# 20171130/Equivariant-NN-Zoo

Measured on AMD Instinct MI355X. Metric: molecules/s forward+backward, QM9 config_energy batch, higher is better.
Workload: dtype f32

## Files before the change

equivariant-nn-zoo_amd/csrc/e3k_layer.hip:

```cpp
#include <cstdlib>
#include <cstring>
#include <new>
#include <vector>

#include "e3k_common.h"

namespace e3k {

__global__ __launch_bounds__(256) void gather_rows_kernel(const float* __restrict__ src, const int64_t* __restrict__ rows, int n_rows,
                                                          int width, float* __restrict__ dst) {
  const int i = blockIdx.x * 256 + threadIdx.x;
  if (i >= n_rows * width) return;
  const int r = i / width, c = i - r * width;
  dst[i] = src[rows[r] * width + c];
}

__global__ __launch_bounds__(256) void scatter_rows_kernel(const float* __restrict__ src, const int64_t* __restrict__ rows,
                                                           const int32_t* __restrict__ bounds, int n_rows, int width,
                                                           float* __restrict__ dst) {
  const int i = blockIdx.x * 256 + threadIdx.x;
  if (i >= n_rows * width) return;
  const int r = i / width, c = i - r * width;
  if (bounds[2 * r + 1] > 0) atomicAdd(dst + rows[r] * width + c, src[i]);
}
// ... 139 lines not shown
    g.add(L, LAST_FWD, r.h, r.w_last, r.use_table ? r.T : r.w, r.R);
    E3K_TRY(g.run(0, st));
  }
  if (r.use_table && !in_kernel_table(d, r)) {
    Timed t(L, E3K_PROF_RTABLE_FWD, st, r.R, r.E);
    E3K_TRY(e3k_rtable_interp_fwd(r.T, r.bin_perm, r.bin, r.bin_coef, r.E, r.knots, d.W, r.w, st));
  }
  return pack_table(L, r, st);
}

}

extern "C" int e3k_layer_create(const e3k_layer_desc* desc, e3k_layer** out) {
  if (!desc || !out || !desc->tp) return E3K_ERR_INVALID;
  if (desc->n_hidden < 1 || desc->n_hidden > 4) return E3K_ERR_UNSUPPORTED;
  if (desc->w_live < 0 || desc->n_live < 0 || desc->n_live > 8 || (desc->w_live > 0) != (desc->n_live > 0)) return E3K_ERR_INVALID;
  if (desc->w_live > 0) {
    if (!e3k_tp_scalar_supported(desc->tp) || (desc->w_live % 4) || desc->w_live > desc->W) return E3K_ERR_UNSUPPORTED;
    int sum = 0;
    for (int i = 0; i < desc->n_live; ++i) {
      if (desc->live_col[i] < 0 || desc->live_len[i] <= 0 || desc->live_col[i] + desc->live_len[i] > desc->W) return E3K_ERR_INVALID;
      sum += desc->live_len[i];
    }
    if (sum != desc->w_live) return E3K_ERR_INVALID;
  }
  e3k_layer* L = new (std::nothrow) e3k_layer();
  if (!L) return E3K_ERR_LAUNCH;
  L->d = *desc;
  const e3k_gemm_set* src[N_SETS] = {&desc->lin1_fwd, &desc->lin1_dgrad, &desc->lin1_dgrad_acc, &desc->lin1_wgrad, &desc->post_fwd,
                                     &desc->post_dgrad, &desc->post_wgrad, &desc->sc_fwd, &desc->sc_dgrad, &desc->sc_wgrad,
                                     &desc->last_fwd, &desc->last_dgrad, &desc->last_wgrad};
  for (int i = 0; i < N_SETS; ++i) {
    const e3k_gemm_set& gs = *src[i];
// ... 219 lines not shown
    }
    if (with_lin1 && need_lin1) g.add(L, LIN1_WGRAD, a->x_cf, a->gb_lin1, a->g_x1, a->N);
    return g.run(1, st, rider);
  };
  if (side3 != main && (need_post || want_sc)) {
    E3K_TRY(edge(L, 0, main, side3));
    E3K_TRY(weight_grads(true, false, side3));
    if (want_sc) E3K_TRY(keyed_weight_grads());
  }
  const bool fused_xw_s = a->fuse_xw && !fused_xw && need_x1 && !in_kernel_table(d, r) && need_radial_side && a->E > 0 && a->g_w && a->x1 &&
                          r.w && side == main;
  const bool rtable_timed = L->prof_cap > 0 && ((L->prof_mask >> E3K_PROF_RTABLE_BWD) & 1u);
  float* const g_T_rows = narrow ? a->g_T_live : a->g_T;
  auto spread_table_gradient = [&](void* st) -> int {
    if (!narrow) return E3K_OK;
    int32_t src_col[8];
    for (int i = 0, pos = 0; i < d.n_live; ++i) {
      src_col[i] = pos;
      pos += d.live_len[i];
    }
    return e3k_expand_columns(a->g_T_live, r.R, d.w_live, d.W, src_col, d.live_col, d.live_len, d.n_live, a->g_T, st);
  };
  const bool ride = fused_xw && r.use_table && side == main && side3 == main && !rtable_timed && a->g_T && a->table_ws &&
                    (r.have_rows || !(need_last || need_hidden || a->need_radial));
  if (need_x1) {
    if (!a->g_x1) return E3K_ERR_INVALID;
    if (!d.tp_bwd_x_overwrites && e3k::zero_fill(a->g_x1, sizeof(float) * a->N * d.d_x1, (hipStream_t)main))
      return E3K_ERR_LAUNCH;
    Timed t(L, E3K_PROF_TP_BWD_X, main, a->N, a->E);
    if (narrow) {
      E3K_TRY(e3k_tp_bwd_xw_scalar_ptable(d.tp, a->x1, r.P, d.W, d.live_col, r.erec_src, a->g_mid, a->src_ptr, a->N, a->E, a->g_x1, a->g_w,
                                          main));
    } else if (fused_xw) {
      E3K_TRY(e3k_tp_bwd_xw_ptable(d.tp, a->x1, r.P, r.erec_src, a->g_mid, a->src_ptr, a->N, a->E, a->g_x1, a->g_w, main));
    } else if (fused_xw_s) {
      E3K_TRY(e3k_tp_bwd_xw(d.tp, a->x1, a->sh, r.w, a->g_mid, a->dst, a->src_ptr, a->src_perm, a->N, a->E, a->g_x1, a->g_w, main));
    } else if (in_kernel_table(d, r) && r.P) {
      E3K_TRY(e3k_tp_bwd_x_ptable(d.tp, r.P, r.erec_src, a->g_mid, a->src_ptr, a->N, a->E, a->g_x1, main));
    } else if (in_kernel_table(d, r)) {
      E3K_TRY(e3k_tp_bwd_x_table(d.tp, a->sh, r.T, r.bin, r.bin_coef, a->g_mid, a->dst, a->src_ptr, a->src_perm, a->N, a->E, a->g_x1, main));
    } else {
      E3K_TRY(e3k_tp_bwd_x(d.tp, a->sh, r.w, a->g_mid, a->dst, a->src_ptr, a->src_perm, a->N, a->E, a->g_x1, main));
    }
  }
  if (need_radial_side && a->E > 0) {
    if (!a->g_w) return E3K_ERR_INVALID;
// ... 248 lines not shown
```

equivariant-nn-zoo_amd/csrc/e3k_tp_scalar.hip:

```cpp
#include "e3k_tp_body.h"

namespace e3k {

constexpr int kScalarMaxGroups = 8;
struct ScalarCols {
  int32_t w_live;
  int32_t table_off[kScalarMaxGroups];
};
template <int L1> struct ScalarSlot { static constexpr int Q = L1 == 0 ? 0 : (L1 == 1 ? 1 : 4); };
static_assert(Slots<0>::L2[ScalarSlot<0>::Q] == 0 && Slots<0>::L3[ScalarSlot<0>::Q] == 0, "slot table changed");
static_assert(Slots<1>::L2[ScalarSlot<1>::Q] == 1 && Slots<1>::L3[ScalarSlot<1>::Q] == 0, "slot table changed");
static_assert(Slots<2>::L2[ScalarSlot<2>::Q] == 2 && Slots<2>::L3[ScalarSlot<2>::Q] == 0, "slot table changed");

template <int L1>
__device__ __forceinline__ void tp_bwd_xw_scalar_body(const TpArgs& a, const e3k_tp_group& g, const int w_live, const int table_off,
                                                      const int node, const int u) {
  constexpr int D1 = 2 * L1 + 1, Q = ScalarSlot<L1>::Q;
  const int mul = g.mul;
  const int u4 = u * 4;
  const int goff4 = uniform(g.out_off[Q] * 4), woff4 = uniform(g.w_off[Q] * 4), toff4 = uniform(table_off * 4);
  const float cf = g.coeff[Q];
  const int row_g = a.d_mid * 4, row_t = a.W * 4, row_w = w_live * 4;
  float gx[D1], xs[D1];
  const float* __restrict__ xr = a.x + (int64_t)node * a.d_in + g.x_off;
// ... 31 lines not shown
#pragma unroll
  for (int i = 0; i < D1; ++i) (gxr + i * mul)[u] = gx[i];
}

__global__ __launch_bounds__(256) void tp_bwd_xw_scalar_kernel(TpArgs a, ScalarCols cols, const e3k_tp_group* __restrict__ groups,
                                                               const int2* __restrict__ gc, int n_gc) {
  E3K_TP_PROLOGUE
  (void)part;
  const int toff = cols.table_off[uniform(gcv.x)];
  const int l1 = g.l1;
  if (l1 == 0) tp_bwd_xw_scalar_body<0>(a, g, cols.w_live, toff, node, u);
  else if (l1 == 1) tp_bwd_xw_scalar_body<1>(a, g, cols.w_live, toff, node, u);
  else tp_bwd_xw_scalar_body<2>(a, g, cols.w_live, toff, node, u);
}

constexpr int kExpandMaxRanges = 8;
struct ExpandRanges {
  int32_t n;
  int32_t src[kExpandMaxRanges], dst[kExpandMaxRanges], len[kExpandMaxRanges];
};
__global__ __launch_bounds__(256) void expand_columns_kernel(const float* __restrict__ src, int64_t rows, int w_src, int w_dst,
                                                             ExpandRanges rg, float* __restrict__ dst) {
  const int q_dst = w_dst / 4;
  const int64_t i = (int64_t)blockIdx.x * 256 + threadIdx.x;
  if (i >= rows * q_dst) return;
  const int64_t r = i / q_dst;
  const int c = (int)(i - r * q_dst) * 4;
  float4 v = make_float4(0.f, 0.f, 0.f, 0.f);
  for (int k = 0; k < rg.n; ++k)
    if (c >= rg.dst[k] && c < rg.dst[k] + rg.len[k]) v = *reinterpret_cast<const float4*>(src + r * w_src + rg.src[k] + (c - rg.dst[k]));
  *reinterpret_cast<float4*>(dst + r * w_dst + c) = v;
// ... 81 lines not shown
```

equivariant-nn-zoo_amd/e3_layers_amd/backend/conv_native.py:

```python
from __future__ import annotations

import ctypes as C
import dataclasses
from typing import List, Optional

import torch

from .tuning import knob as _knob
from torch.autograd.function import once_differentiable

from . import lib as L
from . import memo, ops, radial_table

ENABLED = TP_TABLE_PACKED = TP_BWD_FUSED = 1
PROF_KINDS = {"tp_fwd": 0, "tp_bwd_x": 1, "tp_bwd_w": 2, "rtable_fwd": 3, "rtable_bwd": 4, "radial_last_fwd": 5}
_LAYERS: List["NativeLayer"] = []


MAX_ROUNDS = 4
LIVE_GRAD = _knob("E3K_LIVE_GRAD")
NARROW_MAX_GROUPS = 8


def _hits(lo: int, hi: int, ranges) -> bool:
    return any(lo < b and a < hi for a, b in ranges)


def _covers(instr, width: int) -> bool:
    return sum(w for _, w in {(ins.in_off, ins.mul_in * ins.dim) for ins in instr}) == width


@dataclasses.dataclass
class LiveSets:
    cols: tuple
    conv: list
    post: list
# ... 134 lines not shown
            w += [(g.w_off[q], g.mul) for q in live_q]
            if live_q:
                x1.append((g.x_off, g.x_off + (2 * g.l1 + 1) * g.mul))
        lin1 = [ins for ins in plan.lin1_spec.instr if _hits(ins.out_off, ins.out_off + ins.mul_out * ins.dim, x1)]
        return LiveSets(tuple(cols), conv, post, sc, mid, slots, w, sorted(set(x1)), lin1)

    def narrow(self, cols) -> Optional["NativeLayer"]:
        cols = tuple(cols)
        if cols in self.narrows:
            return self.narrows[cols]
        from ..nn.core import tp_slots

        plan, nl = self.plan, None
        ls = self.live_sets(cols)
        groups = plan.tp_plan.groups
        fits = (0 < len(ls.slots) <= NARROW_MAX_GROUPS and len({gi for gi, _ in ls.slots}) == len(ls.slots) and not plan.addend
                and all(tp_slots(groups[gi].l1)[q] == (groups[gi].l1, 0) and groups[gi].l1 <= 2 and groups[gi].mul % 64 == 0
                        for gi, q in ls.slots))
        if fits:
            live_groups, pos = [], 0
            for gi, q in ls.slots:
                g, n = groups[gi], L.TpGroup()
                n.l1, n.x_off, n.mul, n.mask = g.l1, g.x_off, g.mul, 1 << q
                for t in range(4):
                    n.y_off[t] = g.y_off[t]
                n.w_off[q], n.out_off[q], n.out_stride[q], n.coeff[q] = pos, g.out_off[q], g.out_stride[q], g.coeff[q]
                pos += g.mul
                live_groups.append(n)
            tp = plan.tp_plan
            pruned = dict(tp_plan=ops.TpPlan(live_groups, tp.d_in, tp.d_sh, pos, tp.d_mid),
                          post_spec=dataclasses.replace(plan.post_spec, instr=ls.post, in_covered=_covers(ls.post, plan.post_spec.d_in)),
                          lin1_spec=dataclasses.replace(plan.lin1_spec, instr=ls.lin1, in_covered=_covers(ls.lin1, plan.lin1_spec.d_in)))
            if plan.sc_spec is not None:
                live_sc = [ins for _, ins in ls.sc]
                pruned.update(sc_spec=dataclasses.replace(plan.sc_spec, instr=live_sc, in_covered=_covers(live_sc, plan.sc_spec.d_in)),
                              sc_m_off=tuple(plan.sc_m_off[j] for j, _ in ls.sc))
            np_ = plan.replace(**pruned)
            try:
                nl = NativeLayer(np_, narrow_of=self)
            except NotImplementedError:
                nl = None
        if nl is not None:
            d = nl.desc
            if plan.sc_spec is not None:
                kw = ops._kw_array(plan.sc_spec, plan.sc_m_off)
                nl.keep.append(kw)
                d.kw, d.n_kw = kw, len(plan.sc_spec.instr)
            d.post_in_covered = 1
            d.w_live, d.n_live = pos, len(ls.slots)
            for i, (off, mul) in enumerate(ls.w):
                d.live_col[i], d.live_len[i] = off, mul
            nl.live = ls
        self.narrows[cols] = nl
        return nl

    def _all(self):
        return [self] + [n for n in self.narrows.values() if n is not None]

    def profile(self, capacity: int, kinds=None) -> None:
        mask = 0xFFFFFFFF if kinds is None else sum(1 << PROF_KINDS[k] for k in kinds)
        for lay in self._all():
            lay.prof = (capacity, mask)
            for h in lay.handles.values():
                L.check(L.load().e3k_layer_profile_mask(h, capacity, mask), "e3k_layer_profile_mask")

    def profile_read(self, kind: str):
        out = []
# ... 535 lines not shown
                                  p_tab)
            ctx.cfg = (plan, topo, groups, bool(in_cf), bool(out_cf), fork, len(w_hidden), table, carve, rcarve, need_relayout)
            ctx.stack = stack
            ctx.attrs_shape = tuple(node_attrs.shape) if (has_sc and not have_m) else None
        ctx.addend_inplace = addend_inplace
        if addend_inplace:
            return y, addend
        return y

    @staticmethod
    def backward(ctx, gy, *unused):
        from . import conv_block

        plan, topo, groups, in_cf, out_cf, fork, n_hidden, table, carve, rcarve, need_relayout = ctx.cfg
        live_cols = memo.recall(gy, "live_cols") if (LIVE_GRAD and gy is not None) else None
        saved = ctx.saved_tensors
        x_in, edge_radial, sh, buf, rbuf, w, w_lin1, w_post, w_sc, w_last, t_keep, m_pre = saved[:12]
        conv_ext = None
        if ctx.addend_inplace:
            conv_ext, m_pre = m_pre, None
            if gy is None:
                gy = torch.zeros(conv_ext.shape[0], plan.gate_spec.out_dim, device=conv_ext.device, dtype=torch.float32)
        w_hidden = saved[12:12 + n_hidden]
        p_tab = saved[12 + n_hidden]
        need = ctx.needs_input_grad
        need_x, need_attrs, need_radial, need_sh = need[0], need[1], need[2], need[3]
        stack, need_pre = ctx.stack, need[12]
        have_m, need_m = m_pre is not None, need[13]
        need_addend = bool(plan.addend and need[13])
        p0 = 14
        need_lin1, need_post, need_sc, need_last = need[p0], need[p0 + 1], need[p0 + 2], need[p0 + 3]
        need_hidden = need[p0 + 4:]
        if stack:
            need_radial = need_last = False
            need_hidden = ()
        if torch.is_grad_enabled() or need_sh:
            raise RuntimeError(
                "the fused convolution block serves first-order training only (no gradient w.r.t. the spherical harmonics, "
                "no create_graph=True): MessagePassing takes the composed path for those by itself; set E3K_CONV_BLOCK=0 "
                "if this was reached another way")
        has_sc = plan.sc_spec is not None
        dev = gy.device
        n, e, r = gy.shape[0], sh.shape[0], edge_radial.shape[0]
        narrow = None
        if live_cols is not None:
            cand = native_layer(plan).narrow(live_cols)
            if cand is not None:
                cand.handle(dev)
                if (stack and need_pre and table is not None and p_tab is not None and w is None and (need_x or need_lin1) and e > 0
                        and gy.dtype == torch.float32 and gy.is_contiguous()):
                    narrow = cand
        layer = (narrow or native_layer(plan)).handle(dev)
        main = ops.current_stream(dev)
        fork = fork and not torch.cuda.is_current_stream_capturing()
        side = ops.side_stream(dev, 0) if fork else main
        side2 = ops.side_stream(dev, 1) if fork else main
        side3 = ops.side_stream(dev, 2) if (fork and ops.WGRAD_SIDE) else main
        gy = L.f32c(gy)
        lin1, post, last, sc = plan.lin1_spec, plan.post_spec, plan.last_spec, plan.sc_spec
        off = carve.off
        a = L.LayerBwdArgs()
        a.N, a.E = n, e
        a.in_cf, a.out_cf, a.fork = int(in_cf), int(out_cf), int(fork)
        a.need_x, a.need_attrs, a.need_radial = int(need_x), int(bool(need_attrs and has_sc)), int(need_radial)
        a.fuse_xw = 1
# ... 121 lines not shown
            with conv_block._on(side2, main):
                g_attrs = torch.empty(ctx.attrs_shape, device=dev, dtype=torch.float32)
            a.g_attrs = g_attrs.data_ptr()
        if need_radial:
            with conv_block._on(side, main):
                g_radial = torch.empty_like(edge_radial)
            a.g_radial = g_radial.data_ptr()
        if HOST_TIMING is not None:
            import time

            t_c = time.perf_counter()
            L.check(L.load().e3k_layer_bwd(layer, C.byref(a)), "e3k_layer_bwd")
            HOST_TIMING[3] += time.perf_counter() - t_c
        else:
            L.check(L.load().e3k_layer_bwd(layer, C.byref(a)), "e3k_layer_bwd")
        if fork:
            for st in (side, side2, side3):
                if st is not main:
                    work.record_stream(st)
            buf.record_stream(side)
            if side3 is not main:
                buf.record_stream(side3)
                if x_in is not None:
                    x_in.record_stream(side3)
            _record_once(sh, side)
        if "post" in rets or "lin1" in rets:
            conv_block._wait(main, side3)
        if "sc" in rets:
            conv_block._wait(main, side2)
        if "last" in rets or any(f"h{i}" in rets for i in range(n_hidden)):
# ... 15 lines not shown
```

equivariant-nn-zoo_amd/e3_layers_amd/backend/lib.py:

```python
from __future__ import annotations

import ctypes as C
import os
from typing import Optional, Sequence

import torch

from .tuning import knob as _knob

_HERE = os.path.dirname(os.path.abspath(__file__))
CSRC_DIR = os.path.normpath(os.path.join(_HERE, "..", "..", "csrc"))
LIB_PATH = _knob("E3K_LIB") or os.path.join(CSRC_DIR, "libe3k.so")

TP_MAXQ = 8


class GemmProblem(C.Structure):
    _fields_ = [
        ("A", C.c_void_p), ("A2", C.c_void_p), ("B", C.c_void_p), ("C", C.c_void_p), ("bias", C.c_void_p),
        ("row_index", C.c_void_p), ("group_dev", C.c_void_p),
        ("M1", C.c_int32), ("M2", C.c_int32), ("N", C.c_int32), ("K", C.c_int32),
        ("V", C.c_int32), ("accumulate", C.c_int32),
        ("a_r1", C.c_int64), ("a_r2", C.c_int64), ("a_k", C.c_int64),
        ("a2_r1", C.c_int64),
        ("b_k", C.c_int64), ("b_n", C.c_int64),
        ("c_r1", C.c_int64), ("c_r2", C.c_int64), ("c_n", C.c_int64),
        ("alpha", C.c_float), ("act", C.c_int32), ("act_cst", C.c_float), ("chain", C.c_int32),
    ]

# ... 35 lines not shown
    _fields_ = [("p", C.POINTER(GemmProblem)), ("n", C.c_int32), ("n_rounds", C.c_int32), ("round_start", C.c_int32 * 5),
                ("_pad", C.c_int32)]


class LayerDesc(C.Structure):
    _fields_ = ([("tp", C.c_void_p)]
                + [(k, GemmSet) for k in ("lin1_fwd", "lin1_dgrad", "lin1_dgrad_acc", "lin1_wgrad", "post_fwd", "post_dgrad",
                                          "post_wgrad", "sc_fwd", "sc_dgrad", "sc_wgrad", "last_fwd", "last_dgrad", "last_wgrad")]
                + [("gate", C.POINTER(GateSeg)), ("n_gate", C.c_int32), ("n_in_blocks", C.c_int32), ("in_blocks", C.POINTER(Block)),
                   ("kw", C.POINTER(KwInstr)), ("n_kw", C.c_int32), ("V", C.c_int32), ("ld_m", C.c_int64),
                   ("k0", C.c_int32), ("h", C.c_int32), ("n_hidden", C.c_int32), ("act", C.c_int32), ("cst", C.c_float),
                   ("alphas", C.c_float * 4)]
                + [(k, C.c_int32) for k in ("d_in", "d_x1", "d_mid", "d_conv", "d_out", "W", "post_in_covered", "sc_in_covered",
                                            "lin1_in_covered", "sc_out_covered", "post_out_covered", "tp_bwd_x_overwrites",
                                            "w_live", "n_live")]
                + [("live_col", C.c_int32 * 8), ("live_len", C.c_int32 * 8)])


class LayerRadial(C.Structure):
    _fields_ = [("R", C.c_int64), ("E", C.c_int64), ("use_table", C.c_int32), ("keep", C.c_int32), ("knots", C.c_int32),
                ("have_rows", C.c_int32), ("in_kernel", C.c_int32), ("packed", C.c_int32), ("radial", C.c_void_p), ("bin", C.c_void_p), ("bin_ptr", C.c_void_p), ("bin_perm", C.c_void_p),
                ("bin_coef", C.c_void_p), ("bin_seg", C.c_void_p), ("w_last", C.c_void_p), ("w_hidden", C.c_void_p * 4), ("h", C.c_void_p),
                ("z", C.c_void_p * 4), ("T", C.c_void_p), ("w", C.c_void_p), ("erec_dst", C.c_void_p), ("erec_src", C.c_void_p), ("P", C.c_void_p)]


class RadialStackItem(C.Structure):
    _fields_ = [("rad", LayerRadial), ("g_rows", C.c_void_p), ("gb_last", C.c_void_p), ("gb_hidden", C.c_void_p * 4),
                ("g_h", C.c_void_p), ("g_radial", C.c_void_p), ("g_slope", C.c_void_p), ("hp", C.c_void_p), ("g_hp", C.c_void_p)]


class SlopeCtx(C.Structure):
# ... 121 lines not shown
    "e3k_tp_plan_destroy": (None, [_P]),
    "e3k_tp_fwd": (C.c_int, [_P, _P, _P, _P, _P, _P, _P, _I64, _I64, _P, _P]),
    "e3k_tp_bwd_w": (C.c_int, [_P, _P, _P, _P, _P, _P, _P, _P, _I64, _I64, _P, _P, _P]),
    "e3k_tp_bwd_w_ordered": (C.c_int, [_P, _P, _P, _P, _P, _P, _P, _P, _I64, _I64, _P, _P, _P, _P]),
    "e3k_tp_bwd_x_overwrites": (C.c_int, [_P]),
    "e3k_tp_last_route": (C.c_char_p, []),
    "e3k_gemm_last_routes": (C.c_char_p, []),
    "e3k_tp_table_supported": (C.c_int, [_P]),
    "e3k_tp_fwd_table": (C.c_int, [_P, _P, _P, _P, _P, _P, _P, _P, _P, _I64, _I64, _P, _P]),
    "e3k_tp_bwd_x_table": (C.c_int, [_P, _P, _P, _P, _P, _P, _P, _P, _P, _I64, _I64, _P, _P]),
    "e3k_tp_fwd_ptable": (C.c_int, [_P, _P, _P, _P, _P, _I64, _I64, _P, _P]),
    "e3k_tp_bwd_x_ptable": (C.c_int, [_P, _P, _P, _P, _P, _I64, _I64, _P, _P]),
    "e3k_tp_bwd_xw_ptable": (C.c_int, [_P, _P, _P, _P, _P, _P, _I64, _I64, _P, _P, _P]),
    "e3k_tp_scalar_supported": (C.c_int, [_P]),
    "e3k_tp_bwd_xw_scalar_ptable": (C.c_int, [_P, _P, _P, _I32, C.POINTER(_I32), _P, _P, _P, _I64, _I64, _P, _P, _P]),
    "e3k_expand_columns": (C.c_int, [_P, _I64, _I32, _I32, C.POINTER(_I32), C.POINTER(_I32), C.POINTER(_I32), _I32, _P, _P]),
    "e3k_tp_bwd_xw": (C.c_int, [_P, _P, _P, _P, _P, _P, _P, _P, _I64, _I64, _P, _P, _P]),
    "e3k_tp_bwd_xe": (C.c_int, [_P, _P, _P, _P, _P, _P, _P, _P, _P, _I64, _I64, _P, _P, _P, _P, _P, _P]),
    "e3k_tp_edge_partials_floats": (C.c_int64, [_P, _I64]),
    "e3k_tp_bwd_xw_dual": (C.c_int, [_P, _P, _P, _P, _P, _P, _P, _P, _P, _P, _P, _P, _I64, _I64, _P, _P, _P, _P]),
    "e3k_edge_records": (C.c_int, [_P, _P, _P, _P, _P, _I32, _I64, _P, _P]),
    "e3k_tp_table2_supported": (C.c_int, [_P]),
    "e3k_tp_second_order_streamed_supported": (C.c_int, [_P]),
    "e3k_tp_bwd_e_table": (C.c_int, [_P, _P, _P, _P, _P, _P, _P, _P, _P, _P, _P, _I64, _I64, _P, _P, _P, _P, _P]),
    "e3k_tp_fwd_jvp_table": (C.c_int, [_P, _P, _P, _P, _P, _P, _P, _P, _P, _P, _P, _P, _P, _I64, _I64, _P, _P]),
    "e3k_tp_bwd_x_dual_table": (C.c_int, [_P, _P, _P, _P, _P, _P, _P, _P, _P, _P, _P, _P, _I64, _I64, _P, _P]),
    "e3k_tp_bwd_w_dual": (C.c_int, [_P, _P, _P, _P, _P, _P, _P, _P, _P, _I64, _I64, _P, _P]),
    "e3k_tp_bwd_x": (C.c_int, [_P, _P, _P, _P, _P, _P, _P, _I64, _I64, _P, _P]),
    "e3k_csr_workspace_ints": (C.c_int64, [_I64, _I64]),
    "e3k_csr_build": (C.c_int, [_P, _I64, _I64, _P, _P, _P, _P, _P, _P, _P, _P, _P]),
# ... 118 lines not shown
```

equivariant-nn-zoo_amd/e3_layers_amd/backend/tuning.py:

```python
from __future__ import annotations

import os
from typing import Dict, Tuple

KNOBS: Dict[str, Tuple[object, str, str]] = {
    "E3K_CONV_BLOCK": (1, "path", "a layer as one autograd node (backend/conv_block.py); 0: one autograd.Function per kernel (the definition)"),
    "E3K_FORCE_BLOCK": (1, "path", "force training: a layer as three autograd nodes on the value + slope tables (backend/conv_force.py); 0: composed per-edge path"),
    "E3K_GEMM_CHAIN": (1, "path", "a Linear's terms that add onto one block (an irrep feeding two outputs: the second was an accumulating launch of its own) run as ONE K-chained GEMM problem; 0: one round of launches per term"),
    "E3K_FORCE_EDGE_ATOMICS": (0, "path", "force block: 1 = g_sh / g_r accumulated with float atomics across a plan's groups (rounds 4-5: forces not bit-reproducible); 0 = per-item partials combined in a fixed order"),
    "E3K_BLOCK_ADDEND": (1, "path", "layers with un-keyed node attributes run as fused blocks with the self-connection handed in as addend"),
    "E3K_BLOCK_LOOK_AHEAD": (1, "path", "a forked layer issues the next layer's radial branch behind its own tensor product"),
    "E3K_CF_CHAIN": (1, "path", "consecutive MessagePassing layers hand their features over channel-fastest"),
    "E3K_RADIAL_STACK": (1, "path", "the radial MLPs of all layers on one edge embedding evaluated as one batch"),
    "E3K_KW_STACK": (1, "path", "the per-key self-connection weights of all layers formed as one batch"),
    "E3K_TP_TABLE": (1, "path", "table layers interpolate their path weights inside the tensor-product kernels, from the table packed into 12-byte Taylor records (no w[E, W]); 0: interpolation pass"),
    "E3K_LIVE_GRAD": (1, "path", "a layer whose incoming gradient is marked zero outside some columns (the Linear in front of a scalar head marks it) runs the backward of the live paths only (conv_native.NativeLayer.narrow); 0: always the dense backward"),
    "E3K_FWD_FORK": (1, "path", "0: one stream; 1: radial / self-connection / weight-gradient branches on side streams above the edge thresholds (never inside a graph capture)"),
    "E3K_WGRAD_SIDE": (1, "path", "sunk weight gradients of forked layers run on a side stream"),
    "E3K_FORK_MIN_EDGES": (25000, "threshold", "per-edge radial layers fork from this many edges (in units of a 1920-weight layer)"),
    "E3K_FORK_MIN_EDGES_TABLE": (60000, "threshold", "table layers fork from this many edges"),
    "E3K_STACK_MAX_EDGES": (50000, "threshold", "forked layers use the radial stack up to this many edges (one-stream layers: always)"),
    "E3K_KW_STACK_MAX_EDGES": (10 ** 9, "threshold", "keyed-weight stack up to this many edges (measured: no upper limit pays)"),
    "E3K_WGRAD_SIDE_MIN_ROWS": (2048, "threshold", "composed path: weight gradients move to the side stream from this many rows"),
    "E3K_KEY_MAX": (256, "threshold", "keyed self-connection for at most this many distinct attribute rows"),
    "E3K_RADIAL_TABLE": (1, "accuracy", "radial MLP on a knot table + cubic interpolation per edge (bound by the guard below); 0: per edge"),
    "E3K_RADIAL_KNOTS": (512, "accuracy", "target knot count over [0, r_max] (the spacing is the power of two at or below r_max / knots)"),
    "E3K_RADIAL_KNOTS_SLOPE": (512, "accuracy", "... of the value + slope tables of force training"),
    "E3K_RADIAL_KNOTS_MAX": (2048, "accuracy", "a guard whose bound passes the tolerance doubles both knot counts up to this; beyond it that MLP's table is switched off (= E3K_RADIAL_KNOTS: never refine)"),
    "E3K_RADIAL_TABLE_KEYED": (0, "path", "one knot table per value of a small categorical edge key beside the radius (config_diffusion's bond type); measured slower than the per-edge MLP for the 32-channel net it serves: off"),
    "E3K_RADIAL_MIN_EDGES_PER_KNOT": (4.0, "threshold", "the table applies from this many edges per table row"),
    "E3K_RADIAL_TABLE_TOL": (1e-6, "accuracy", "a-posteriori interpolation-error bound above which an MLP's table is switched off"),
# ... 39 lines not shown
```

include/e3k.h:

```cpp
#ifndef E3K_H
#define E3K_H

#include <stdint.h>

#ifdef __cplusplus
extern "C" {
#endif

#define E3K_OK 0
#define E3K_ERR_INVALID (-1)
#define E3K_ERR_LAUNCH (-2)
#define E3K_ERR_UNSUPPORTED (-3)

#define E3K_TP_MAXQ 8

const char* e3k_strerror(int code);
int e3k_version(void);
void e3k_tp_limits(int* l1max, int* l2max, int* l3max);

typedef struct {
  const float* A;
  const float* A2;
  const float* B;
  float* C;
  const float* bias;
  const int32_t* row_index;
  const int32_t* group_dev;
  int32_t M1, M2, N, K;
  int32_t V;
// ... 105 lines not shown
int e3k_tp_table_supported(const e3k_tp_plan* plan);
int e3k_tp_fwd_table(const e3k_tp_plan* plan, const float* x, const float* sh, const float* T, const int32_t* bin,
                     const float* coef, const int32_t* src, const int32_t* dst_ptr, const int32_t* dst_perm, int64_t N, int64_t E,
                     float* out, void* stream);
int e3k_tp_bwd_x_table(const e3k_tp_plan* plan, const float* sh, const float* T, const int32_t* bin, const float* coef,
                       const float* g_out, const int32_t* dst, const int32_t* src_ptr, const int32_t* src_perm, int64_t N,
                       int64_t E, float* g_x, void* stream);
int e3k_tp_fwd_ptable(const e3k_tp_plan* plan, const float* x, const void* P, const int32_t* erec_dst, const int32_t* dst_ptr,
                      int64_t N, int64_t E, float* out, void* stream);
int e3k_tp_bwd_x_ptable(const e3k_tp_plan* plan, const void* P, const int32_t* erec_src, const float* g_out, const int32_t* src_ptr,
                        int64_t N, int64_t E, float* g_x, void* stream);
int e3k_tp_bwd_xw_ptable(const e3k_tp_plan* plan, const float* x, const void* P, const int32_t* erec_src, const float* g_out,
                         const int32_t* src_ptr, int64_t N, int64_t E, float* g_x, float* g_w, void* stream);
int e3k_tp_scalar_supported(const e3k_tp_plan* plan);
int e3k_tp_bwd_xw_scalar_ptable(const e3k_tp_plan* plan, const float* x, const void* P, int32_t table_w, const int32_t* table_off,
                                const int32_t* erec_src, const float* g_out, const int32_t* src_ptr, int64_t N, int64_t E, float* g_x,
                                float* g_w, void* stream);
int e3k_expand_columns(const float* src, int64_t rows, int32_t w_src, int32_t w_dst, const int32_t* src_col, const int32_t* dst_col,
                       const int32_t* len, int32_t n_ranges, float* dst, void* stream);
int e3k_tp_bwd_xw(const e3k_tp_plan* plan, const float* x, const float* sh, const float* w, const float* g_out, const int32_t* dst,
                  const int32_t* src_ptr, const int32_t* src_perm, int64_t N, int64_t E, float* g_x, float* g_w, void* stream);
int e3k_tp_table2_supported(const e3k_tp_plan* plan);
int e3k_tp_second_order_streamed_supported(const e3k_tp_plan* plan);
int e3k_tp_bwd_e_table(const e3k_tp_plan* plan, const float* x, const float* sh, const float* T, const float* D,
                       const int32_t* bin, const float* coef, const float* g_out, const int32_t* src, const int32_t* dst_ptr,
                       const int32_t* dst_perm, int64_t N, int64_t E, float* g_sh, float* g_r, float* g_w, float* e_partials,
                       void* stream);
int64_t e3k_tp_edge_partials_floats(const e3k_tp_plan* plan, int64_t E);
int e3k_tp_fwd_jvp_table(const e3k_tp_plan* plan, const float* x, const float* x2, const float* sh, const float* sh2,
                         const float* T, const float* D, const int32_t* bin, const float* coef, const float* s2,
// ... 281 lines not shown
  e3k_gemm_set sc_fwd, sc_dgrad, sc_wgrad;
  e3k_gemm_set last_fwd, last_dgrad, last_wgrad;
  const e3k_gate_seg* gate;
  int32_t n_gate;
  int32_t n_in_blocks;
  const e3k_block* in_blocks;
  const e3k_kw_instr* kw;
  int32_t n_kw, V;
  int64_t ld_m;
  int32_t k0, h, n_hidden, act;
  float cst;
  float alphas[4];
  int32_t d_in, d_x1, d_mid, d_conv, d_out, W;
  int32_t post_in_covered, sc_in_covered, lin1_in_covered, sc_out_covered, post_out_covered, tp_bwd_x_overwrites;
  int32_t w_live, n_live;
  int32_t live_col[8], live_len[8];
} e3k_layer_desc;

typedef struct e3k_layer e3k_layer;
int e3k_layer_create(const e3k_layer_desc* desc, e3k_layer** out);
void e3k_layer_destroy(e3k_layer* layer);

typedef struct {
  int64_t R, E;
  int32_t use_table, keep, knots;
  int32_t have_rows;
  int32_t in_kernel;
  int32_t packed;
  const float* radial;
  const int32_t* bin;
  const int32_t* bin_ptr;
// ... 114 lines not shown
```

Measured before the change: 84910.

## Extend live-path narrow backward to multi-slot masked groups and propagate live columns

Adds a masked tensor-product backward kernel that computes input and weight gradients only for the live output slots of each group, including non-scalar L3<=2 paths, instead of the full dense backward. A layer that ran narrow now records which of its input columns carry gradient, so the preceding layer can also take the narrow path; hint columns are used to build narrow plans early. The slot limit is raised to 48 and adjacent column ranges are merged before expansion. This adds a more complex eligibility rule (the live share must be at most 75% of the rows) and extra branching per slot inside the kernel.

```diff
diff --git a/equivariant-nn-zoo_amd/csrc/e3k_layer.hip b/equivariant-nn-zoo_amd/csrc/e3k_layer.hip
--- a/equivariant-nn-zoo_amd/csrc/e3k_layer.hip
+++ b/equivariant-nn-zoo_amd/csrc/e3k_layer.hip
@@ -177,9 +177,11 @@
 extern "C" int e3k_layer_create(const e3k_layer_desc* desc, e3k_layer** out) {
   if (!desc || !out || !desc->tp) return E3K_ERR_INVALID;
   if (desc->n_hidden < 1 || desc->n_hidden > 4) return E3K_ERR_UNSUPPORTED;
-  if (desc->w_live < 0 || desc->n_live < 0 || desc->n_live > 8 || (desc->w_live > 0) != (desc->n_live > 0)) return E3K_ERR_INVALID;
+  if (desc->w_live < 0 || desc->n_live < 0 || desc->n_live > E3K_NARROW_MAX_SLOTS || (desc->w_live > 0) != (desc->n_live > 0))
+    return E3K_ERR_INVALID;
   if (desc->w_live > 0) {
-    if (!e3k_tp_scalar_supported(desc->tp) || (desc->w_live % 4) || desc->w_live > desc->W) return E3K_ERR_UNSUPPORTED;
+    if (!(e3k_tp_scalar_supported(desc->tp) || e3k_tp_masked_supported(desc->tp)) || (desc->w_live % 4) || desc->w_live > desc->W)
+      return E3K_ERR_UNSUPPORTED;
     int sum = 0;
     for (int i = 0; i < desc->n_live; ++i) {
       if (desc->live_col[i] < 0 || desc->live_len[i] <= 0 || desc->live_col[i] + desc->live_len[i] > desc->W) return E3K_ERR_INVALID;
@@ -429,12 +431,17 @@
   float* const g_T_rows = narrow ? a->g_T_live : a->g_T;
   auto spread_table_gradient = [&](void* st) -> int {
     if (!narrow) return E3K_OK;
-    int32_t src_col[8];
-    for (int i = 0, pos = 0; i < d.n_live; ++i) {
-      src_col[i] = pos;
-      pos += d.live_len[i];
-    }
-    return e3k_expand_columns(a->g_T_live, r.R, d.w_live, d.W, src_col, d.live_col, d.live_len, d.n_live, a->g_T, st);
+    int32_t src_col[E3K_NARROW_MAX_SLOTS], dst_col[E3K_NARROW_MAX_SLOTS], len[E3K_NARROW_MAX_SLOTS];
+    int n = 0;
+    for (int i = 0, pos = 0; i < d.n_live; pos += d.live_len[i], ++i) {
+      if (n && dst_col[n - 1] + len[n - 1] == d.live_col[i]) {
+        len[n - 1] += d.live_len[i];
+      } else {
+        src_col[n] = pos; dst_col[n] = d.live_col[i]; len[n] = d.live_len[i];
+        ++n;
+      }
+    }
+    return e3k_expand_columns(a->g_T_live, r.R, d.w_live, d.W, src_col, dst_col, len, n, a->g_T, st);
   };
   const bool ride = fused_xw && r.use_table && side == main && side3 == main && !rtable_timed && a->g_T && a->table_ws &&
                     (r.have_rows || !(need_last || need_hidden || a->need_radial));
@@ -443,8 +450,11 @@
     if (!d.tp_bwd_x_overwrites && e3k::zero_fill(a->g_x1, sizeof(float) * a->N * d.d_x1, (hipStream_t)main))
       return E3K_ERR_LAUNCH;
     Timed t(L, E3K_PROF_TP_BWD_X, main, a->N, a->E);
-    if (narrow) {
+    if (narrow && e3k_tp_scalar_supported(d.tp)) {
       E3K_TRY(e3k_tp_bwd_xw_scalar_ptable(d.tp, a->x1, r.P, d.W, d.live_col, r.erec_src, a->g_mid, a->src_ptr, a->N, a->E, a->g_x1, a->g_w,
+                                          main));
+    } else if (narrow) {
+      E3K_TRY(e3k_tp_bwd_xw_masked_ptable(d.tp, a->x1, r.P, d.W, d.live_col, r.erec_src, a->g_mid, a->src_ptr, a->N, a->E, a->g_x1, a->g_w,
                                           main));
     } else if (fused_xw) {
       E3K_TRY(e3k_tp_bwd_xw_ptable(d.tp, a->x1, r.P, r.erec_src, a->g_mid, a->src_ptr, a->N, a->E, a->g_x1, a->g_w, main));
diff --git a/equivariant-nn-zoo_amd/csrc/e3k_tp_masked.hip b/equivariant-nn-zoo_amd/csrc/e3k_tp_masked.hip
--- /dev/null
+++ b/equivariant-nn-zoo_amd/csrc/e3k_tp_masked.hip
@@ -0,0 +1,179 @@
+#include "e3k_tp_body.h"
+
+namespace e3k {
+
+constexpr int kMaskedMaxGroups = 8;
+constexpr int kMaskedL3Max = 2;
+struct MaskedCols {
+  int32_t w_live;
+  int32_t table_off[kMaskedMaxGroups][E3K_MAXQ];
+};
+
+template <int L1>
+__device__ __forceinline__ void tp_bwd_xw_masked_body(const TpArgs& a, const e3k_tp_group& g, const MaskedCols& cols, const int gi,
+                                                      const int node, const int u) {
+  using S = Slots<L1>;
+  constexpr int D1 = 2 * L1 + 1, L3MAX = kMaskedL3Max;
+  const int mul = g.mul;
+  const int u4 = u * 4;
+  const unsigned mask = uniform(g.mask);
+  const int row_g = a.d_mid * 4, row_t = a.W * 4, row_w = cols.w_live * 4;
+  int goff4[S::NQ], gstr4[S::NQ], woff4[S::NQ], toff4[S::NQ];
+  float cf[S::NQ];
+  slot_for_part<S, L1, L3MAX, 2>([&](auto qc) {
+    constexpr int Q = decltype(qc)::value;
+    goff4[Q] = uniform(g.out_off[Q] * 4);
+    gstr4[Q] = uniform(g.out_stride[Q] * 4);
+    woff4[Q] = uniform(g.w_off[Q] * 4);
+    toff4[Q] = uniform(cols.table_off[gi][Q] * 4);
+    cf[Q] = g.coeff[Q];
+  });
+  float gx[D1], xs[D1];
+  const float* __restrict__ xr = a.x + (int64_t)node * a.d_in + g.x_off;
+#pragma unroll
+  for (int i = 0; i < D1; ++i) {
+    gx[i] = 0.0f;
+    xs[i] = (xr + i * mul)[u];
+  }
+  const int beg = uniform(a.ptr[node]), end = uniform(a.ptr[node + 1]);
+  EdgeRec cur{};
+  if (beg < end) cur = load_rec(a.erec, beg);
+  for (int t = beg; t < end; ++t) {
+    const EdgeRec nxt = load_rec(a.erec, t + 1 < end ? t + 1 : t);
+    YRegs yc;
+    rec_y(yc, cur);
+    const __amdgpu_buffer_rsrc_t rg = row_rsrc(a.g_out + (int64_t)cur.nbr * a.d_mid, row_g);
+    const __amdgpu_buffer_rsrc_t rgw = row_rsrc(a.g_w + (int64_t)cur.e * cols.w_live, row_w);
+    const KnotPacked kp = knot_packed_rec(a, cur, row_t * 3);
+    float gn[S::TOTAL];
+    PackedRec rec[S::NQ];
+    slot_for_part<S, L1, L3MAX, 2>([&](auto qc) {
+      constexpr int Q = decltype(qc)::value;
+      constexpr int L3 = S::L3[Q], OFF = S::OFF[Q];
+      if (mask & (1u << Q)) {
+#pragma unroll
+        for (int k = 0; k < 2 * L3 + 1; ++k)
+          gn[OFF + k] = buf_ld(rg, u4, goff4[Q] + k * gstr4[Q]);
+        rec[Q] = buf_ld_rec(kp.r, u4, toff4[Q], row_t * 2);
+      } else {
+#pragma unroll
+        for (int k = 0; k < 2 * L3 + 1; ++k) gn[OFF + k] = 0.0f;
+      }
+    });
+    __builtin_amdgcn_sched_barrier(0);
+    float wn[S::NQ];
+    slot_for_part<S, L1, L3MAX, 2>([&](auto qc) {
+      constexpr int Q = decltype(qc)::value;
+      wn[Q] = packed_mix(kp, rec[Q]);
+    });
+    slot_for_part<S, L1, L3MAX, 2>([&](auto qc) {
+      constexpr int Q = decltype(qc)::value;
+      constexpr int L2 = S::L2[Q], L3 = S::L3[Q], OFF = S::OFF[Q];
+      if (mask & (1u << Q)) {
+        float gk[2 * L3 + 1];
+#pragma unroll
+        for (int k = 0; k < 2 * L3 + 1; ++k) gk[k] = gn[OFF + k];
+        float tq[D1];
+        CG<L1, L2, L3>::yt(yref<L2>(yc), gk, tq);
+        const float sw = wn[Q] * cf[Q];
+        float dot = 0.0f;
+#pragma unroll
+        for (int i = 0; i < D1; ++i) {
+          gx[i] = fmaf(sw, tq[i], gx[i]);
+          dot = fmaf(xs[i], tq[i], dot);
+        }
+        buf_st_stream(dot * cf[Q], rgw, u4, woff4[Q]);
+      }
+    });
+    cur = nxt;
+  }
+  float* __restrict__ gxr = a.g_x + (int64_t)node * a.d_in + g.x_off;
+#pragma unroll
+  for (int i = 0; i < D1; ++i) {
+    if (!a.x_shared) (gxr + i * mul)[u] = gx[i];
+    else atomicAdd(gxr + i * mul + u, gx[i]);
+  }
+}
+
+__global__ __launch_bounds__(256, 8) void tp_bwd_xw_masked_kernel(TpArgs a, MaskedCols cols, const e3k_tp_group* __restrict__ groups,
+                                                                  const int2* __restrict__ gc, int n_gc) {
+  E3K_TP_PROLOGUE
+  (void)part;
+  const int gi = uniform(gcv.x);
+  const int l1 = g.l1;
+  if (l1 == 0) tp_bwd_xw_masked_body<0>(a, g, cols, gi, node, u);
+  else if (l1 == 1) tp_bwd_xw_masked_body<1>(a, g, cols, gi, node, u);
+  else tp_bwd_xw_masked_body<2>(a, g, cols, gi, node, u);
+}
+
+namespace {
+int masked_slot_l3(int l1, int q) {
+  if (q < 0) return -1;
+  if (l1 == 0) return q < Slots<0>::NQ ? Slots<0>::L3[q] : -1;
+  if (l1 == 1) return q < Slots<1>::NQ ? Slots<1>::L3[q] : -1;
+  return q < Slots<2>::NQ ? Slots<2>::L3[q] : -1;
+}
+}
+
+}
+
+extern "C" int e3k_tp_masked_supported(const e3k_tp_plan* p) {
+  if (!p || !p->h_groups || p->n_groups > e3k::kMaskedMaxGroups || p->split || p->d_sh != 9) return 0;
+  for (int i = 0; i < p->n_groups; ++i) {
+    const e3k_tp_group& g = p->h_groups[i];
+    if (g.l1 < 0 || g.l1 > 2 || g.mul <= 0 || g.mul % 64 || !g.mask) return 0;
+    if (g.y_off[0] != 0 || g.y_off[1] != 1 || g.y_off[2] != 4) return 0;
+    if (g.x_off < 0 || g.x_off + (2 * g.l1 + 1) * g.mul > p->d_in) return 0;
+    for (int q = 0; q < E3K_MAXQ; ++q) {
+      if (!((g.mask >> q) & 1u)) continue;
+      const int l3 = e3k::masked_slot_l3(g.l1, q);
+      if (l3 < 0 || l3 > e3k::kMaskedL3Max) return 0;
+      if (g.out_off[q] < 0 || g.out_stride[q] < 0 || (int64_t)g.out_off[q] + 2 * l3 * (int64_t)g.out_stride[q] + g.mul > p->d_mid) return 0;
+      if (g.w_off[q] < 0 || g.w_off[q] + g.mul > p->w_numel) return 0;
+    }
+  }
+  return 1;
+}
+
+extern "C" int e3k_tp_bwd_xw_masked_ptable(const e3k_tp_plan* plan, const float* x, const void* P, int32_t table_w,
+                                           const int32_t* live_col, const int32_t* erec_src, const float* g_out,
+                                           const int32_t* src_ptr, int64_t N, int64_t E, float* g_x, float* g_w, void* stream) {
+  if (!plan || N < 0 || E < 0) return E3K_ERR_INVALID;
+  if (!e3k_tp_masked_supported(plan)) return E3K_ERR_UNSUPPORTED;
+  if (N == 0) return E3K_OK;
+  if (!x || !g_out || !g_x || !src_ptr || (E > 0 && (!P || !erec_src || !g_w))) return E3K_ERR_INVALID;
+  if (reinterpret_cast<uintptr_t>(erec_src) & 63) return E3K_ERR_UNSUPPORTED;
+  if (live_col ? table_w <= 0 : table_w != 0) return E3K_ERR_INVALID;
+  const int tw = live_col ? table_w : plan->w_numel;
+  if ((int64_t)tw * 12 > 0x7fffffffLL) return E3K_ERR_UNSUPPORTED;
+  e3k::MaskedCols cols{};
+  cols.w_live = plan->w_numel;
+  for (int i = 0, k = 0; i < plan->n_groups; ++i) {
+    const e3k_tp_group& g = plan->h_groups[i];
+    for (int q = 0; q < E3K_MAXQ; ++q) {
+      if (!((g.mask >> q) & 1u)) continue;
+      const int col = live_col ? live_col[k] : g.w_off[q];
+      ++k;
+      if (col < 0 || col + g.mul > tw) return E3K_ERR_INVALID;
+      cols.table_off[i][q] = col;
+    }
+  }
+  const int n_gc = plan->n_gc;
+  e3k::TpArgs a{};
+  a.d_in = plan->d_in; a.d_sh = plan->d_sh; a.d_mid = plan->d_mid;
+  a.W = tw;
+  a.ptr = src_ptr;
+  a.x = x; a.w = static_cast<const float*>(P); a.erec = erec_src; a.g_out = g_out; a.g_x = g_x; a.g_w = g_w;
+  a.x_shared = plan->x_shared;
+  a.n_items = N * n_gc;
+  a.order = N >= 64 ? 1 : 0;
+  int64_t blocks = (a.n_items + 3) / 4;
+  if (a.order) blocks = 8 * ((((N + 7) / 8) * n_gc + 3) / 4);
+  if (blocks > 0x7fffffffLL) return E3K_ERR_INVALID;
+  if (blocks == 0) return E3K_OK;
+  e3k::tp_record_route("tp_bwd_xw_masked_kernel");
+  hipLaunchKernelGGL(e3k::tp_bwd_xw_masked_kernel, dim3((unsigned)blocks), dim3(256), 0, (hipStream_t)stream, a, cols, plan->d_groups,
+                     plan->d_gc, n_gc);
+  E3K_CHECK_LAUNCH();
+  return E3K_OK;
+}
diff --git a/equivariant-nn-zoo_amd/csrc/e3k_tp_scalar.hip b/equivariant-nn-zoo_amd/csrc/e3k_tp_scalar.hip
--- a/equivariant-nn-zoo_amd/csrc/e3k_tp_scalar.hip
+++ b/equivariant-nn-zoo_amd/csrc/e3k_tp_scalar.hip
@@ -69,7 +69,7 @@
   else tp_bwd_xw_scalar_body<2>(a, g, cols.w_live, toff, node, u);
 }
 
-constexpr int kExpandMaxRanges = 8;
+constexpr int kExpandMaxRanges = E3K_NARROW_MAX_SLOTS;
 struct ExpandRanges {
   int32_t n;
   int32_t src[kExpandMaxRanges], dst[kExpandMaxRanges], len[kExpandMaxRanges];
diff --git a/equivariant-nn-zoo_amd/e3_layers_amd/backend/conv_native.py b/equivariant-nn-zoo_amd/e3_layers_amd/backend/conv_native.py
--- a/equivariant-nn-zoo_amd/e3_layers_amd/backend/conv_native.py
+++ b/equivariant-nn-zoo_amd/e3_layers_amd/backend/conv_native.py
@@ -20,6 +20,13 @@
 MAX_ROUNDS = 4
 LIVE_GRAD = _knob("E3K_LIVE_GRAD")
 NARROW_MAX_GROUPS = 8
+NARROW_MAX_SLOTS = L.NARROW_MAX_SLOTS
+NARROW_MAX_SHARE = 0.75
+
+
+def live_input_cols(ls: "LiveSets") -> tuple:
+    ins_all = list(ls.lin1) + [ins for _, ins in ls.sc]
+    return tuple(sorted({(ins.in_off, ins.in_off + ins.mul_in * ins.dim) for ins in ins_all}))
 
 
 def _hits(lo: int, hi: int, ranges) -> bool:
@@ -184,20 +191,39 @@
         plan, nl = self.plan, None
         ls = self.live_sets(cols)
         groups = plan.tp_plan.groups
-        fits = (0 < len(ls.slots) <= NARROW_MAX_GROUPS and len({gi for gi, _ in ls.slots}) == len(ls.slots) and not plan.addend
-                and all(tp_slots(groups[gi].l1)[q] == (groups[gi].l1, 0) and groups[gi].l1 <= 2 and groups[gi].mul % 64 == 0
-                        for gi, q in ls.slots))
+        tp = plan.tp_plan
+        usable = bool(ls.slots) and not plan.addend and all(groups[gi].l1 <= 2 and groups[gi].mul % 64 == 0 for gi, _ in ls.slots)
+        scalar = (usable and len(ls.slots) <= NARROW_MAX_GROUPS and len({gi for gi, _ in ls.slots}) == len(ls.slots)
+                  and all(tp_slots(groups[gi].l1)[q] == (groups[gi].l1, 0) for gi, q in ls.slots))
+        rows_live = sum(2 * tp_slots(groups[gi].l1)[q][1] + 1 for gi, q in ls.slots)
+        rows_all = sum(2 * l3 + 1 for g in groups for q, (_, l3) in enumerate(tp_slots(g.l1)) if (g.mask >> q) & 1)
+        masked = (usable and not scalar and len({gi for gi, _ in ls.slots}) <= NARROW_MAX_GROUPS and len(ls.slots) <= NARROW_MAX_SLOTS
+                  and tp.d_sh == 9 and all(tp_slots(groups[gi].l1)[q][1] <= 2 and tuple(groups[gi].y_off[:3]) == (0, 1, 4)
+                                           for gi, q in ls.slots)
+                  and rows_live <= NARROW_MAX_SHARE * rows_all)
+        fits = scalar or masked
         if fits:
             live_groups, pos = [], 0
-            for gi, q in ls.slots:
-                g, n = groups[gi], L.TpGroup()
-                n.l1, n.x_off, n.mul, n.mask = g.l1, g.x_off, g.mul, 1 << q
-                for t in range(4):
-                    n.y_off[t] = g.y_off[t]
-                n.w_off[q], n.out_off[q], n.out_stride[q], n.coeff[q] = pos, g.out_off[q], g.out_stride[q], g.coeff[q]
-                pos += g.mul
-                live_groups.append(n)
-            tp = plan.tp_plan
+            if scalar:
+                for gi, q in ls.slots:
+                    g, n = groups[gi], L.TpGroup()
+                    n.l1, n.x_off, n.mul, n.mask = g.l1, g.x_off, g.mul, 1 << q
+                    for t in range(4):
+                        n.y_off[t] = g.y_off[t]
+                    n.w_off[q], n.out_off[q], n.out_stride[q], n.coeff[q] = pos, g.out_off[q], g.out_stride[q], g.coeff[q]
+                    pos += g.mul
+                    live_groups.append(n)
+            else:
+                for gi in sorted({gi for gi, _ in ls.slots}):
+                    g, n = groups[gi], L.TpGroup()
+                    n.l1, n.x_off, n.mul, n.mask = g.l1, g.x_off, g.mul, 0
+                    for t in range(4):
+                        n.y_off[t] = g.y_off[t]
+                    for q in [q for gj, q in ls.slots if gj == gi]:
+                        n.mask |= 1 << q
+                        n.w_off[q], n.out_off[q], n.out_stride[q], n.coeff[q] = pos, g.out_off[q], g.out_stride[q], g.coeff[q]
+                        pos += g.mul
+                    live_groups.append(n)
             pruned = dict(tp_plan=ops.TpPlan(live_groups, tp.d_in, tp.d_sh, pos, tp.d_mid),
                           post_spec=dataclasses.replace(plan.post_spec, instr=ls.post, in_covered=_covers(ls.post, plan.post_spec.d_in)),
                           lin1_spec=dataclasses.replace(plan.lin1_spec, instr=ls.lin1, in_covered=_covers(ls.lin1, plan.lin1_spec.d_in)))
@@ -221,6 +247,7 @@
             for i, (off, mul) in enumerate(ls.w):
                 d.live_col[i], d.live_len[i] = off, mul
             nl.live = ls
+            nl.form = "scalar" if scalar else "masked"
         self.narrows[cols] = nl
         return nl
 
@@ -786,6 +813,7 @@
 
         plan, topo, groups, in_cf, out_cf, fork, n_hidden, table, carve, rcarve, need_relayout = ctx.cfg
         live_cols = memo.recall(gy, "live_cols") if (LIVE_GRAD and gy is not None) else None
+        hint_cols = memo.recall(gy, "live_cols_hint") if (LIVE_GRAD and gy is not None and live_cols is None) else None
         saved = ctx.saved_tensors
         x_in, edge_radial, sh, buf, rbuf, w, w_lin1, w_post, w_sc, w_last, t_keep, m_pre = saved[:12]
         conv_ext = None
@@ -814,13 +842,13 @@
         has_sc = plan.sc_spec is not None
         dev = gy.device
         n, e, r = gy.shape[0], sh.shape[0], edge_radial.shape[0]
-        narrow = None
-        if live_cols is not None:
-            cand = native_layer(plan).narrow(live_cols)
+        narrow = cand = None
+        if live_cols is not None or hint_cols is not None:
+            cand = native_layer(plan).narrow(live_cols if live_cols is not None else hint_cols)
             if cand is not None:
                 cand.handle(dev)
-                if (stack and need_pre and table is not None and p_tab is not None and w is None and (need_x or need_lin1) and e > 0
-                        and gy.dtype == torch.float32 and gy.is_contiguous()):
+                if (live_cols is not None and stack and need_pre and table is not None and p_tab is not None and w is None
+                        and (need_x or need_lin1) and e > 0 and gy.dtype == torch.float32 and gy.is_contiguous()):
                     narrow = cand
         layer = (narrow or native_layer(plan)).handle(dev)
         main = ops.current_stream(dev)
@@ -972,6 +1000,10 @@
             HOST_TIMING[3] += time.perf_counter() - t_c
         else:
             L.check(L.load().e3k_layer_bwd(layer, C.byref(a)), "e3k_layer_bwd")
+        if narrow is not None and g_x is not None:
+            memo.remember(g_x, "live_cols", live_input_cols(narrow.live))
+        elif cand is not None and g_x is not None:
+            memo.remember(g_x, "live_cols_hint", live_input_cols(cand.live))
         if fork:
             for st in (side, side2, side3):
                 if st is not main:
diff --git a/equivariant-nn-zoo_amd/e3_layers_amd/backend/lib.py b/equivariant-nn-zoo_amd/e3_layers_amd/backend/lib.py
--- a/equivariant-nn-zoo_amd/e3_layers_amd/backend/lib.py
+++ b/equivariant-nn-zoo_amd/e3_layers_amd/backend/lib.py
@@ -13,6 +13,7 @@
 LIB_PATH = _knob("E3K_LIB") or os.path.join(CSRC_DIR, "libe3k.so")
 
 TP_MAXQ = 8
+NARROW_MAX_SLOTS = 48
 
 
 class GemmProblem(C.Structure):
@@ -78,7 +79,7 @@
                 + [(k, C.c_int32) for k in ("d_in", "d_x1", "d_mid", "d_conv", "d_out", "W", "post_in_covered", "sc_in_covered",
                                             "lin1_in_covered", "sc_out_covered", "post_out_covered", "tp_bwd_x_overwrites",
                                             "w_live", "n_live")]
-                + [("live_col", C.c_int32 * 8), ("live_len", C.c_int32 * 8)])
+                + [("live_col", C.c_int32 * NARROW_MAX_SLOTS), ("live_len", C.c_int32 * NARROW_MAX_SLOTS)])
 
 
 class LayerRadial(C.Structure):
@@ -230,6 +231,8 @@
     "e3k_tp_bwd_xw_ptable": (C.c_int, [_P, _P, _P, _P, _P, _P, _I64, _I64, _P, _P, _P]),
     "e3k_tp_scalar_supported": (C.c_int, [_P]),
     "e3k_tp_bwd_xw_scalar_ptable": (C.c_int, [_P, _P, _P, _I32, C.POINTER(_I32), _P, _P, _P, _I64, _I64, _P, _P, _P]),
+    "e3k_tp_masked_supported": (C.c_int, [_P]),
+    "e3k_tp_bwd_xw_masked_ptable": (C.c_int, [_P, _P, _P, _I32, C.POINTER(_I32), _P, _P, _P, _I64, _I64, _P, _P, _P]),
     "e3k_expand_columns": (C.c_int, [_P, _I64, _I32, _I32, C.POINTER(_I32), C.POINTER(_I32), C.POINTER(_I32), _I32, _P, _P]),
     "e3k_tp_bwd_xw": (C.c_int, [_P, _P, _P, _P, _P, _P, _P, _P, _I64, _I64, _P, _P, _P]),
     "e3k_tp_bwd_xe": (C.c_int, [_P, _P, _P, _P, _P, _P, _P, _P, _P, _I64, _I64, _P, _P, _P, _P, _P, _P]),
diff --git a/equivariant-nn-zoo_amd/e3_layers_amd/backend/tuning.py b/equivariant-nn-zoo_amd/e3_layers_amd/backend/tuning.py
--- a/equivariant-nn-zoo_amd/e3_layers_amd/backend/tuning.py
+++ b/equivariant-nn-zoo_amd/e3_layers_amd/backend/tuning.py
@@ -14,7 +14,7 @@
     "E3K_RADIAL_STACK": (1, "path", "the radial MLPs of all layers on one edge embedding evaluated as one batch"),
     "E3K_KW_STACK": (1, "path", "the per-key self-connection weights of all layers formed as one batch"),
     "E3K_TP_TABLE": (1, "path", "table layers interpolate their path weights inside the tensor-product kernels, from the table packed into 12-byte Taylor records (no w[E, W]); 0: interpolation pass"),
-    "E3K_LIVE_GRAD": (1, "path", "a layer whose incoming gradient is marked zero outside some columns (the Linear in front of a scalar head marks it) runs the backward of the live paths only (conv_native.NativeLayer.narrow); 0: always the dense backward"),
+    "E3K_LIVE_GRAD": (1, "path", "a layer whose incoming gradient is marked zero outside some columns (the Linear in front of a scalar head marks it, and a layer that ran narrow marks its own input gradient) runs the backward of the live paths only (conv_native.NativeLayer.narrow); 0: always the dense backward"),
     "E3K_FWD_FORK": (1, "path", "0: one stream; 1: radial / self-connection / weight-gradient branches on side streams above the edge thresholds (never inside a graph capture)"),
     "E3K_WGRAD_SIDE": (1, "path", "sunk weight gradients of forked layers run on a side stream"),
     "E3K_FORK_MIN_EDGES": (25000, "threshold", "per-edge radial layers fork from this many edges (in units of a 1920-weight layer)"),
diff --git a/include/e3k.h b/include/e3k.h
--- a/include/e3k.h
+++ b/include/e3k.h
@@ -13,6 +13,7 @@
 #define E3K_ERR_UNSUPPORTED (-3)
 
 #define E3K_TP_MAXQ 8
+#define E3K_NARROW_MAX_SLOTS 48
 
 const char* e3k_strerror(int code);
 int e3k_version(void);
@@ -148,6 +149,10 @@
                          const int32_t* src_ptr, int64_t N, int64_t E, float* g_x, float* g_w, void* stream);
 int e3k_tp_scalar_supported(const e3k_tp_plan* plan);
 int e3k_tp_bwd_xw_scalar_ptable(const e3k_tp_plan* plan, const float* x, const void* P, int32_t table_w, const int32_t* table_off,
+                                const int32_t* erec_src, const float* g_out, const int32_t* src_ptr, int64_t N, int64_t E, float* g_x,
+                                float* g_w, void* stream);
+int e3k_tp_masked_supported(const e3k_tp_plan* plan);
+int e3k_tp_bwd_xw_masked_ptable(const e3k_tp_plan* plan, const float* x, const void* P, int32_t table_w, const int32_t* live_col,
                                 const int32_t* erec_src, const float* g_out, const int32_t* src_ptr, int64_t N, int64_t E, float* g_x,
                                 float* g_w, void* stream);
 int e3k_expand_columns(const float* src, int64_t rows, int32_t w_src, int32_t w_dst, const int32_t* src_col, const int32_t* dst_col,
@@ -459,7 +464,7 @@
   int32_t d_in, d_x1, d_mid, d_conv, d_out, W;
   int32_t post_in_covered, sc_in_covered, lin1_in_covered, sc_out_covered, post_out_covered, tp_bwd_x_overwrites;
   int32_t w_live, n_live;
-  int32_t live_col[8], live_len[8];
+  int32_t live_col[E3K_NARROW_MAX_SLOTS], live_len[E3K_NARROW_MAX_SLOTS];
 } e3k_layer_desc;
 
 typedef struct e3k_layer e3k_layer;
```

Measured after the change: 91740 (median of 6 runs). 1.08x the previous value.
